# rlorenzo/facet

Hardware: AMD Instinct MI355X
Metric: images/sec whole-node (TOPIQ+SAMP+CLIP+InsightFace ensemble), 1024² batch (higher is better)
Workload: dtype f32

## Files before the change

### facet_amd/csrc/capi.hip

```cpp
#include "capi_internal.h"

static std::string g_create_err;

extern "C" {

const char* fe_version(void) { return "facet_amd 0.1 (gfx950)"; }

int fe_create(int device, size_t arena_bytes, fe_ctx** out) {
  if (!out) return FE_ERR_INVALID;
  *out = nullptr;
  try {
    int ndev = 0;
    hipError_t e = hipGetDeviceCount(&ndev);
    if (e != hipSuccess || ndev <= 0) throw Error(std::string("no HIP device available: ") + hipGetErrorString(e));
    FE_CHECK(device >= 0 && device < ndev, "device %d out of range (%d devices)", device, ndev);
    FE_HIP(hipSetDevice(device));
    hipDeviceProp_t prop;
    FE_HIP(hipGetDeviceProperties(&prop, device));
    FE_CHECK(std::string(prop.gcnArchName).rfind("gfx950", 0) == 0, "device %d is %s; this engine is built for gfx950 only",
             device, prop.gcnArchName);
    auto* x = new fe_ctx();
    x->c.device = device;
    FE_HIP(hipStreamCreateWithFlags(&x->c.stream, hipStreamNonBlocking));
    if (!arena_bytes) {
      size_t free_b = 0, total_b = 0;
      FE_HIP(hipMemGetInfo(&free_b, &total_b));
      arena_bytes = std::min<size_t>((size_t)64 << 30, std::max<size_t>((size_t)2 << 30, free_b / 4));
    }
    x->c.arena.init(arena_bytes);
    FE_HIP(hipEventCreate(&x->t0));
    FE_HIP(hipEventCreate(&x->t1));
    *out = x;
  } catch (const std::exception& e) {
    g_create_err = e.what();
    return FE_ERR_RUNTIME;
  }
  return FE_OK;
}

void fe_destroy(fe_ctx* ctx) {
  if (!ctx) return;
  (void)hipSetDevice(ctx->c.device);
  (void)hipStreamSynchronize(ctx->c.stream);
  if (ctx->t0) (void)hipEventDestroy(ctx->t0);
  if (ctx->t1) (void)hipEventDestroy(ctx->t1);
  if (ctx->d_out) (void)hipFree(ctx->d_out);
  if (ctx->d_rec) (void)hipFree(ctx->d_rec);
  for (int i = 0; i < 2; ++i) {
    if (ctx->stage_buf[i]) (void)hipFree(ctx->stage_buf[i]);
    if (ctx->ev_copied[i]) (void)hipEventDestroy(ctx->ev_copied[i]);
    if (ctx->ev_consumed[i]) (void)hipEventDestroy(ctx->ev_consumed[i]);
  }
  if (ctx->copy_stream) (void)hipStreamDestroy(ctx->copy_stream);
  for (void* q : ctx->misc_allocs) (void)hipFree(q);
  if (ctx->clip_in) (void)hipFree(ctx->clip_in);
  if (ctx->samp_in) (void)hipFree(ctx->samp_in);
  delete ctx;
}

const char* fe_last_error(fe_ctx* ctx) { return ctx ? ctx->c.err.c_str() : g_create_err.c_str(); }

int fe_sync(fe_ctx* ctx) {
  return fe_api(ctx, [&] {
    FE_HIP(hipStreamSynchronize(ctx->c.stream));
  });
}

int fe_set_microbatch(fe_ctx* ctx, int n) {
  return fe_api(ctx, [&] {
    FE_CHECK(n >= 1 && n <= 256, "microbatch %d out of range", n);
    ctx->microbatch = n;
  });
}

int fe_set_conv_variant(fe_ctx* ctx, int variant) {
  return fe_api(ctx, [&] {
    ctx->c.force_variant = variant;
  });
}

int fe_dev_alloc(fe_ctx* ctx, size_t bytes, void** d_out) {
  return fe_api(ctx, [&] {
    FE_CHECK(d_out != nullptr, "null out");
    FE_HIP(hipSetDevice(ctx->c.device));
    FE_HIP(hipMalloc(d_out, bytes ? bytes : 16));
  });
// ... 245 lines not shown
```

### facet_amd/csrc/capi_internal.h

```cpp
#pragma once
#include "../../include/facet_engine.h"
#include "engine.h"
#include "onnx_graph.h"
#include <algorithm>
#include <cmath>
#include <cstring>
#include <stdexcept>
#include <tuple>
#include <type_traits>

using namespace fe;

struct fe_ctx {
  Ctx c;
  int microbatch = 8;
  hipEvent_t t0 = nullptr, t1 = nullptr;
  hipStream_t copy_stream = nullptr;
  uint8_t* stage_buf[2] = {nullptr, nullptr};
  size_t stage_cap[2] = {0, 0};
  hipEvent_t ev_copied[2] = {nullptr, nullptr}, ev_consumed[2] = {nullptr, nullptr};
  short* warp_wtab = nullptr;
  struct CvResizeTab { int* ofs; short* coef; };
  std::map<std::tuple<int, int, int>, CvResizeTab> cvresize;
  int* hsv_sdiv = nullptr; int* hsv_hdiv = nullptr;
  double* phash_cos = nullptr;
  std::vector<void*> misc_allocs;
  float* clip_in = nullptr;
  size_t clip_in_cap = 0;
  float* samp_in = nullptr;
  size_t samp_in_cap = 0;
  float* d_rec = nullptr;
  size_t d_rec_cap = 0;
  int ensemble_mask = 7;
  float* d_out = nullptr;
  size_t d_out_cap = 0;
  float* out_buf(size_t floats) {
    if (floats > d_out_cap) {
      if (d_out) (void)hipFree(d_out);
      d_out = nullptr; d_out_cap = 0;
      FE_HIP(hipMalloc((void**)&d_out, floats * sizeof(float)));
      d_out_cap = floats;
    }
    return d_out;
  }
};

class ImageStager {
 public:
  ImageStager(fe_ctx* ctx, const uint8_t* imgs, int n, size_t per_image, int mb, int on_device)
      : x_(ctx), imgs_(imgs), n_(n), per_(per_image), mb_(mb), dev_(on_device) {
    if (!dev_) {
      if (!x_->copy_stream) {
        FE_HIP(hipStreamCreateWithFlags(&x_->copy_stream, hipStreamNonBlocking));
        for (int i = 0; i < 2; ++i) {
          FE_HIP(hipEventCreateWithFlags(&x_->ev_copied[i], hipEventDisableTiming));
          FE_HIP(hipEventCreateWithFlags(&x_->ev_consumed[i], hipEventDisableTiming));
        }
      }
      const size_t need = (size_t)std::min(mb_, n_) * per_;
      for (int i = 0; i < 2; ++i)
        if (x_->stage_cap[i] < need) {
          FE_HIP(hipStreamSynchronize(x_->c.stream));
          if (x_->stage_buf[i]) FE_HIP(hipFree(x_->stage_buf[i]));
          x_->stage_buf[i] = nullptr; x_->stage_cap[i] = 0;
          FE_HIP(hipMalloc((void**)&x_->stage_buf[i], need));
          x_->stage_cap[i] = need;
        }
      issue(0);
    }
  }
  int chunks() const { return (n_ + mb_ - 1) / mb_; }
  int count(int k) const { return std::min(mb_, n_ - k * mb_); }
  const uint8_t* get(int k) {
    if (dev_) return imgs_ + (size_t)k * mb_ * per_;
    FE_HIP(hipStreamWaitEvent(x_->c.stream, x_->ev_copied[k & 1], 0));
    return x_->stage_buf[k & 1];
  }
  void done(int k) {
    if (dev_) return;
    FE_HIP(hipEventRecord(x_->ev_consumed[k & 1], x_->c.stream));
    consumed_[k & 1] = true;
    if (k + 1 < chunks()) issue(k + 1);
  }
 private:
  void issue(int k) {
    const int b = k & 1;
    if (consumed_[b]) FE_HIP(hipStreamWaitEvent(x_->copy_stream, x_->ev_consumed[b], 0));
    FE_HIP(hipMemcpyAsync(x_->stage_buf[b], imgs_ + (size_t)k * mb_ * per_, (size_t)count(k) * per_, hipMemcpyHostToDevice,
                          x_->copy_stream));
    FE_HIP(hipEventRecord(x_->ev_copied[b], x_->copy_stream));
  }
  fe_ctx* x_; const uint8_t* imgs_; int n_; size_t per_; int mb_, dev_;
  bool consumed_[2] = {false, false};
};

inline void fe_drain(fe_ctx* ctx) {
  if (ctx->copy_stream) (void)hipStreamSynchronize(ctx->copy_stream);
  if (ctx->c.stream) (void)hipStreamSynchronize(ctx->c.stream);
}

struct CapacityError : std::runtime_error { using std::runtime_error::runtime_error; };

enum class OnError {
  Runtime,
  Capacity,
  VlmCapacity
};
inline bool vlm_capacity_error(const char* msg) {
  return strstr(msg, "arena exhausted") || strstr(msg, "out of memory") || strstr(msg, "do not fit") || strstr(msg, "max_seq <= 8192");
}

template <class F>
int fe_api(fe_ctx* ctx, OnError policy, F&& body) {
  if (!ctx) return FE_ERR_INVALID;
  try {
    (void)hipSetDevice(ctx->c.device);
    if constexpr (std::is_void_v<decltype(body())>) {
      body();
      return FE_OK;
    } else {
      return body();
    }
  } catch (const std::exception& e) {
    ctx->c.err = e.what();
    fe_drain(ctx);
    const bool capacity = (policy == OnError::Capacity && dynamic_cast<const CapacityError*>(&e)) ||
                          (policy == OnError::VlmCapacity && vlm_capacity_error(e.what()));
    return capacity ? FE_ERR_CAPACITY : FE_ERR_RUNTIME;
  }
}
template <class F>
int fe_api(fe_ctx* ctx, F&& body) { return fe_api(ctx, OnError::Runtime, body); }
// ... 31 lines not shown
```

### facet_amd/csrc/capi_models.hip

```cpp
#include "capi_internal.h"

namespace {
const float kImagenetMean[3] = {0.485f, 0.456f, 0.406f};
const float kImagenetStd[3] = {0.229f, 0.224f, 0.225f};
const float kClipMean[3] = {0.48145466f, 0.4578275f, 0.40821073f};
const float kClipStd[3] = {0.26862954f, 0.26130258f, 0.27577711f};

int py_round_half_even(double v) {
  const double f = std::floor(v);
  const double d = v - f;
  if (d > 0.5) return (int)f + 1;
  if (d < 0.5) return (int)f;
  return ((long long)f % 2 == 0) ? (int)f : (int)f + 1;
}

template <class T>
void topiq_backbone_chunk(fe_ctx* ctx, const uint8_t* d_rgb, int nb, int h, int w, std::vector<TensorT<T>>& feats) {
  Ctx& C = ctx->c;
  const int long_edge = h > w ? h : w;
  if (long_edge > 1024) {
    const double sc = 1024.0 / long_edge;
    const int nw = (int)(w * sc), nh = (int)(h * sc);
    uint8_t* small = (uint8_t*)C.arena.alloc((size_t)nb * nh * nw * 3);
    resize_u8(C, d_rgb, nb, h, w, nh, nw, FE_FILTER_LANCZOS, 0, nh, 0, nw, small);
    d_rgb = small; h = nh; w = nw;
  }
  Tensor x = C.arena.tensor(nb, h, w, 4);
  launch_u8_to_nhwc4_norm(d_rgb, x.p, (size_t)nb * h * w, kImagenetMean, kImagenetStd, 0, C.stream);
  resnet_forward<T>(C, ctx->c.topiq->backbone, x, &feats, ctx->c.topiq->dw.res32);
}
void topiq_chunk_score(fe_ctx* ctx, const uint8_t* d_in, int nb, int h, int w, float* d_scores) {
  Ctx& C = ctx->c;
  const bool small = (size_t)h * (size_t)w < C.topiq_f32_below && !C.topiq->dw.half_only && !C.topiq->dw.res32;
// ... 36 lines not shown
  auto samp_on = [&](auto sal) {
    typedef decltype(sal.p) SP;
    typedef std::remove_pointer_t<SP> TS;
    if (!with_samp) return;
    if (C.samp->dw.prec == PREC_BF16) sampnet_forward<bf16, TS>(C, *C.samp, x, sal, pw, at, sd);
    else if (C.samp->dw.prec == PREC_F16) sampnet_forward<f16, TS>(C, *C.samp, x, sal, pw, at, sd);
    else sampnet_forward<float, TS>(C, *C.samp, x, sal, pw, at, sd);
  };
  const int prec = C.u2netp->dw.prec;
  if (prec == PREC_BF16) {
    TensorH sal = C.arena.tensor_t<bf16>(x.n, x.h, x.w, 1);
    u2netp_forward<bf16>(C, *C.u2netp, x, sal);
    samp_on(sal);
    if (d_sal) launch_convert(sal.p, d_sal, sal.numel(), C.stream);
  } else if (prec == PREC_F16) {
    TensorF16 sal = C.arena.tensor_t<f16>(x.n, x.h, x.w, 1);
    u2netp_forward<f16>(C, *C.u2netp, x, sal);
    samp_on(sal);
    if (d_sal) launch_convert(sal.p, d_sal, sal.numel(), C.stream);
  } else {
    Tensor sal = C.arena.tensor(x.n, x.h, x.w, 1);
    u2netp_forward<float>(C, *C.u2netp, x, sal);
    samp_on(sal);
    if (d_sal) FE_HIP(hipMemcpyAsync(d_sal, sal.p, sal.numel() * sizeof(float), hipMemcpyDeviceToDevice, C.stream));
  }
}

void compact_crops(float* buf, size_t per, int c, int left, hipStream_t s) {
  for (int done = 0; done < left; done += c) {
    const int n = std::min(c, left - done);
    FE_HIP(hipMemcpyAsync(buf + (size_t)done * per, buf + (size_t)(c + done) * per, (size_t)n * per * sizeof(float), hipMemcpyDeviceToDevice, s));
  }
}
int clip_tower_chunk(const ClipModel& m, int n) {
  if (n <= 40) return n;
  const int hi = std::min(n, 128), lo = std::max(32, hi - 40), ntile = std::max(1, m.width / 128);
  int best = hi;
  double best_eff = 0.0;
  for (int c = hi; c >= lo; --c) {
    const long wgs = (((long)c * m.tokens + 127) / 128) * ntile;
    const double eff = (double)wgs / (double)(((wgs + 255) / 256) * 256);
    if (eff > best_eff + 1e-9) { best_eff = eff; best = c; }
  }
  return best;
}
void clip_tower(Ctx& C, const Tensor& x, float* feat) {
  const bool r32 = C.clip->dw.res32;
  if (C.clip->split3) { clip_forward_split3(C, *C.clip, x, feat); return; }
  if (C.clip->dw.prec == PREC_BF16) { if (r32) clip_forward<bf16, float>(C, *C.clip, x, feat); else clip_forward<bf16>(C, *C.clip, x, feat); }
  else if (C.clip->dw.prec == PREC_F16) { if (r32) clip_forward<f16, float>(C, *C.clip, x, feat); else clip_forward<f16>(C, *C.clip, x, feat); }
  else clip_forward<float>(C, *C.clip, x, feat);
}
class ClipBatcher {
 public:
  ClipBatcher(fe_ctx* ctx, int n_total, int max_push, float* d_feat, float* d_norm, float* d_aes)
      : x_(ctx), feat_(d_feat), norm_(d_norm), aes_(d_aes) {
    const ClipModel& m = *ctx->c.clip;
    hw_ = m.patch_size * (int)std::lround(std::sqrt((double)(m.tokens - 1)));
    od_ = m.out_dim;
    per_ = (size_t)hw_ * hw_ * 4;
    chunk_ = clip_tower_chunk(m, n_total);
    const size_t need = (size_t)(chunk_ + max_push) * per_;
    if (ctx->clip_in_cap < need) {
      FE_HIP(hipStreamSynchronize(ctx->c.stream));
      if (ctx->clip_in) FE_HIP(hipFree(ctx->clip_in));
      ctx->clip_in = nullptr; ctx->clip_in_cap = 0;
      FE_HIP(hipMalloc((void**)&ctx->clip_in, need * sizeof(float)));
      ctx->clip_in_cap = need;
    }
  }
  void push(const Tensor& xt) {
    FE_CHECK(xt.c == 4 && xt.ld == 4 && xt.h == hw_ && xt.w == hw_, "clip batcher: crop layout");
    FE_HIP(hipMemcpyAsync(x_->clip_in + (size_t)count_ * per_, xt.p, (size_t)xt.n * per_ * sizeof(float), hipMemcpyDeviceToDevice, x_->c.stream));
    count_ += xt.n;
    while (count_ >= chunk_) run(chunk_);
  }
  void finish() {
    while (count_ > 0) run(std::min(count_, chunk_));
  }
 private:
  void run(int c) {
    Ctx& C = x_->c;
    const size_t mark = C.arena.mark();
    Tensor x;
    x.p = x_->clip_in; x.n = c; x.h = hw_; x.w = hw_; x.c = 4; x.ld = 4;
    clip_tower(C, x, feat_ + (size_t)done_ * od_);
    if (norm_) l2_normalize(C, feat_ + (size_t)done_ * od_, norm_ + (size_t)done_ * od_, c, od_);
    if (aes_) aesthetic_forward(C, *C.aesthetic, feat_ + (size_t)done_ * od_, c, aes_ + done_);
    C.arena.rewind(mark);
    const int left = count_ - c;
    compact_crops(x_->clip_in, per_, c, left, C.stream);
    done_ += c;
    count_ = left;
  }
  fe_ctx* x_;
  float *feat_, *norm_, *aes_;
  int hw_ = 224, od_ = 768, chunk_ = 1, count_ = 0, done_ = 0;
  size_t per_ = 0;
};
class SampBatcher {
 public:
  SampBatcher(fe_ctx* ctx, int n_total, int max_push, float* pw, float* at, float* sd) : x_(ctx), pw_(pw), at_(at), sd_(sd) {
    const size_t room = ctx->c.arena.capacity() > ((size_t)8 << 30) ? ctx->c.arena.capacity() - ((size_t)8 << 30) : ctx->c.arena.capacity() / 4;
    const int fit = (int)std::min<size_t>(128, std::max<size_t>(1, room / ((size_t)150 << 20)));
    chunk_ = std::max(1, std::min(n_total, std::max(fit, std::min(max_push, 32))));
    per_ = (size_t)224 * 224 * 4;
    const size_t need = (size_t)(chunk_ + max_push) * per_;
    if (ctx->samp_in_cap < need) {
      FE_HIP(hipStreamSynchronize(ctx->c.stream));
      if (ctx->samp_in) FE_HIP(hipFree(ctx->samp_in));
      ctx->samp_in = nullptr; ctx->samp_in_cap = 0;
      FE_HIP(hipMalloc((void**)&ctx->samp_in, need * sizeof(float)));
      ctx->samp_in_cap = need;
    }
  }
  void push(const Tensor& xt) {
    FE_CHECK(xt.c == 4 && xt.ld == 4 && xt.h == 224 && xt.w == 224, "samp batcher: crop layout");
    FE_HIP(hipMemcpyAsync(x_->samp_in + (size_t)count_ * per_, xt.p, (size_t)xt.n * per_ * sizeof(float), hipMemcpyDeviceToDevice, x_->c.stream));
    count_ += xt.n;
    while (count_ >= chunk_) run(chunk_);
  }
  void finish() {
    while (count_ > 0) run(std::min(count_, chunk_));
  }
 private:
  void run(int c) {
    Ctx& C = x_->c;
    const size_t mark = C.arena.mark();
    Tensor x;
    x.p = x_->samp_in; x.n = c; x.h = 224; x.w = 224; x.c = 4; x.ld = 4;
    samp_chunk(x_, x, true, pw_ + (size_t)done_ * 8, at_ + (size_t)done_ * 6, sd_ + (size_t)done_ * 5, nullptr);
    C.arena.rewind(mark);
    const int left = count_ - c;
    compact_crops(x_->samp_in, per_, c, left, C.stream);
    done_ += c;
    count_ = left;
  }
  fe_ctx* x_;
  float *pw_, *at_, *sd_;
  int chunk_ = 1, count_ = 0, done_ = 0;
  size_t per_ = 0;
};

__global__ void records_interleave_kernel(const float* __restrict__ planes, size_t n4, int n, float* __restrict__ rec, int ld) {
  const size_t i = (size_t)blockIdx.x * blockDim.x + threadIdx.x;
  if (i >= (size_t)n * FE_RECORD_FLOATS) return;
  const int img = (int)(i / FE_RECORD_FLOATS), f = (int)(i - (size_t)img * FE_RECORD_FLOATS);
  const size_t o_aes = n4, o_pw = 2 * n4, o_at = o_pw + 8 * n4, o_sd = o_at + 6 * n4, o_emb = o_sd + 5 * n4;
  float v;
  if (f == 0) v = planes[img];
  else if (f == 1) v = planes[o_aes + img];
  else if (f < 10) v = planes[o_pw + (size_t)img * 8 + (f - 2)];
  else if (f < 16) v = planes[o_at + (size_t)img * 6 + (f - 10)];
  else if (f < 21) v = planes[o_sd + (size_t)img * 5 + (f - 16)];
  else v = planes[o_emb + (size_t)img * 768 + (f - 21)];
  rec[(size_t)img * ld + f] = v;
}

int ensemble_run(fe_ctx* ctx, const uint8_t* rgb, int n, int h, int w, int on_device, float* d_rec, int ld) {
  Ctx& C = ctx->c;
  const size_t per = (size_t)h * w * 3;
  const size_t n4 = ((size_t)n + 3) & ~(size_t)3;
  const size_t o_aes = n4, o_pw = 2 * n4, o_at = o_pw + 8 * n4, o_sd = o_at + 6 * n4, o_emb = o_sd + 5 * n4,
               o_feat = o_emb + 768 * n4, total = o_feat + 768 * n4;
  float* d_pl = ctx->out_buf(total);
  FE_HIP(hipMemsetAsync(d_pl, 0, total * sizeof(float), C.stream));
  const int sel = ctx->ensemble_mask;
  const bool do_topiq = (sel & 1) && C.topiq && C.topiq->has_head, do_clip = (sel & 2) && C.clip, do_samp = (sel & 4) && C.samp && C.u2netp;
  float* p_topiq = d_pl;  float* p_aes = d_pl + o_aes;  float* p_pw = d_pl + o_pw;  float* p_at = d_pl + o_at;
  float* p_sd = d_pl + o_sd;  float* p_emb = d_pl + o_emb;  float* d_feat = d_pl + o_feat;
  std::unique_ptr<ClipBatcher> tower;
  if (do_clip) tower = std::make_unique<ClipBatcher>(ctx, n, ctx->microbatch, d_feat, p_emb, C.aesthetic ? p_aes : nullptr);
  std::unique_ptr<SampBatcher> samp;
  if (do_samp) samp = std::make_unique<SampBatcher>(ctx, n, ctx->microbatch, p_pw, p_at, p_sd);
  ImageStager st(ctx, rgb, n, per, ctx->microbatch, on_device);
  for (int k = 0; k < st.chunks(); ++k) {
    const int i0 = k * ctx->microbatch, nb = st.count(k);
    C.arena.reset();
    const uint8_t* d_in = st.get(k);
    if (do_topiq) {
      const size_t mark = C.arena.mark();
      topiq_chunk_score(ctx, d_in, nb, h, w, p_topiq + i0);
      C.arena.rewind(mark);
    }
    if (do_clip) {
      const size_t mark = C.arena.mark();
      Tensor xt = preprocess_square224(C, d_in, nb, h, w, FE_FILTER_BICUBIC, true, kClipMean, kClipStd, 0);
      tower->push(xt);
      C.arena.rewind(mark);
    }
    if (do_samp) {
      const size_t mark = C.arena.mark();
      Tensor xt = preprocess_square224(C, d_in, nb, h, w, FE_FILTER_BILINEAR, false, kImagenetMean, kImagenetStd, 0);
      samp->push(xt);
      C.arena.rewind(mark);
    }
    st.done(k);
  }
  if (tower) tower->finish();
  if (samp) samp->finish();
  const size_t work = (size_t)n * FE_RECORD_FLOATS;
  hipLaunchKernelGGL(records_interleave_kernel, dim3((unsigned)((work + 255) / 256)), dim3(256), 0, C.stream, d_pl, n4, n, d_rec, ld);
  FE_HIP(hipGetLastError());
  return (do_topiq ? 1 : 0) | (do_clip ? 2 : 0) | (do_samp ? 4 : 0);
}
}

extern "C" {

int fe_topiq_feature_shape(int h, int w, int level, int dims[3]) {
  if (!dims || h < 32 || w < 32 || level < 0 || level > 4) return FE_ERR_INVALID;
  const int long_edge = h > w ? h : w;
  if (long_edge > 1024) {
    const double sc = 1024.0 / long_edge;
    w = (int)(w * sc); h = (int)(h * sc);
  }
  static const int ch[5] = {64, 256, 512, 1024, 2048};
  int fh = conv_out_dim(h, 7, 2, 3, 1), fw = conv_out_dim(w, 7, 2, 3, 1);
  if (level >= 1) { fh = conv_out_dim(fh, 3, 2, 1, 1); fw = conv_out_dim(fw, 3, 2, 1, 1); }
  for (int l = 2; l <= level; ++l) { fh = conv_out_dim(fh, 3, 2, 1, 1); fw = conv_out_dim(fw, 3, 2, 1, 1); }
  dims[0] = ch[level]; dims[1] = fh; dims[2] = fw;
  return FE_OK;
}

int fe_topiq_features(fe_ctx* ctx, const uint8_t* rgb, int n, int h, int w, int on_device, int level, float* out) {
  return fe_api(ctx, [&] {
    Ctx& C = ctx->c;
    if (!C.topiq) { C.err = "topiq weights not loaded"; return FE_ERR_NOT_LOADED; }
    FE_CHECK(rgb && out && n > 0 && h >= 32 && w >= 32 && level >= 0 && level <= 4, "bad arguments");
    const size_t img_bytes = (size_t)h * w * 3;
    size_t out_per_img = 0;
    for (int i0 = 0; i0 < n; i0 += ctx->microbatch) {
      const int nb = std::min(ctx->microbatch, n - i0);
      C.arena.reset();
      const uint8_t* d_in = resident(C, rgb + (size_t)i0 * img_bytes, nb * img_bytes, on_device);
      if (C.topiq->dw.prec == PREC_BF16) {
// ... 89 lines not shown
}

int fe_aesthetic_score(fe_ctx* ctx, const float* feats, int n, float* aesthetic_raw) {
  return fe_api(ctx, [&] {
    Ctx& C = ctx->c;
    if (!C.aesthetic) { C.err = "aesthetic head weights not loaded"; return FE_ERR_NOT_LOADED; }
    FE_CHECK(feats && aesthetic_raw && n > 0, "bad arguments");
    const int d = 768;
    for (int i0 = 0; i0 < n; i0 += 65536) {
      const int nb = std::min(65536, n - i0);
      C.arena.reset();
      float* d_in = upload(C, feats + (size_t)i0 * d, (size_t)nb * d);
      float* d_out = (float*)C.arena.alloc((size_t)nb * sizeof(float));
      aesthetic_forward(C, *C.aesthetic, d_in, nb, d_out);
      FE_HIP(hipMemcpyAsync(aesthetic_raw + i0, d_out, (size_t)nb * sizeof(float), hipMemcpyDeviceToHost, C.stream));
      FE_HIP(hipStreamSynchronize(C.stream));
    }
    return FE_OK;
  });
}

int fe_clip_encode_image(fe_ctx* ctx, const float* x, int n, int on_device, float* features, float* emb_norm,
                         float* aesthetic_raw) {
  return fe_api(ctx, [&] {
    Ctx& C = ctx->c;
    if (!C.clip) { C.err = "clip weights not loaded"; return FE_ERR_NOT_LOADED; }
    if (aesthetic_raw && !C.aesthetic) { C.err = "aesthetic head weights not loaded"; return FE_ERR_NOT_LOADED; }
    FE_CHECK(x && n > 0 && (features || emb_norm || aesthetic_raw), "bad arguments");
    const int hw = C.clip->patch_size * (int)std::lround(std::sqrt((double)(C.clip->tokens - 1)));
    const int od = C.clip->out_dim;
    const size_t per = (size_t)3 * hw * hw;
    float* d_out = ctx->out_buf((size_t)n * (2 * od + 1));
    float* d_feat = d_out; float* d_norm = d_out + (size_t)n * od; float* d_aes = d_out + (size_t)n * 2 * od;
    const int step = clip_tower_chunk(*C.clip, n);
    for (int i0 = 0; i0 < n; i0 += step) {
      const int nb = std::min(step, n - i0);
      C.arena.reset();
      Tensor xt;
      if (on_device) {
        xt = C.arena.tensor(nb, hw, hw, 4);
        launch_nchw_to_nhwc(x + (size_t)i0 * per, xt.p, nb, 3, hw, hw, 4, C.stream);
      } else {
        xt = upload_nchw(C, x + (size_t)i0 * per, nb, 3, hw, hw, 4);
      }
      clip_tower(C, xt, d_feat + (size_t)i0 * od);
      if (emb_norm) l2_normalize(C, d_feat + (size_t)i0 * od, d_norm + (size_t)i0 * od, nb, od);
      if (aesthetic_raw) aesthetic_forward(C, *C.aesthetic, d_feat + (size_t)i0 * od, nb, d_aes + i0);
    }
    if (features) FE_HIP(hipMemcpyAsync(features, d_feat, (size_t)n * od * sizeof(float), hipMemcpyDeviceToHost, C.stream));
    if (emb_norm) FE_HIP(hipMemcpyAsync(emb_norm, d_norm, (size_t)n * od * sizeof(float), hipMemcpyDeviceToHost, C.stream));
    if (aesthetic_raw) FE_HIP(hipMemcpyAsync(aesthetic_raw, d_aes, (size_t)n * sizeof(float), hipMemcpyDeviceToHost, C.stream));
    FE_HIP(hipStreamSynchronize(C.stream));
    return FE_OK;
  });
}

int fe_clip_encode_images(fe_ctx* ctx, const uint8_t* rgb, int n, int h, int w, int on_device, float* features,
                          float* emb_norm, float* aesthetic_raw) {
  return fe_api(ctx, [&] {
    Ctx& C = ctx->c;
    if (!C.clip) { C.err = "clip weights not loaded"; return FE_ERR_NOT_LOADED; }
    if (aesthetic_raw && !C.aesthetic) { C.err = "aesthetic head weights not loaded"; return FE_ERR_NOT_LOADED; }
    FE_CHECK(rgb && n > 0 && h > 0 && w > 0, "bad arguments");
    const int od = C.clip->out_dim;
    const size_t per = (size_t)h * w * 3;
    float* d_out = ctx->out_buf((size_t)n * (2 * od + 1));
    float* d_feat = d_out; float* d_norm = d_out + (size_t)n * od; float* d_aes = d_out + (size_t)n * 2 * od;
// ... 130 lines not shown
```

### facet_amd/csrc/fe_common.h

```cpp
#pragma once
#include <hip/hip_runtime.h>
#include "fe_check.h"
#include <cstdint>
#include <cstdio>
#include <atomic>
#include <cstring>
#include <map>
#include <mutex>
#include <stdexcept>
#include <string>
#include <vector>

namespace fe {


#define FE_HIP(expr)                                                                      \
  do {                                                                                    \
    hipError_t _e = (expr);                                                               \
    if (_e != hipSuccess) {                                                               \
      char _b[512];                                                                       \
      snprintf(_b, sizeof _b, "%s:%d: %s -> %s", __FILE__, __LINE__, #expr,               \
               hipGetErrorString(_e));                                                    \
      throw fe::Error(_b);                                                                \
    }                                                                                     \
  } while (0)

inline void ensure_dynamic_lds(const void* kernel, size_t bytes, std::atomic<uint64_t>& done) {
  int dev = 0;
  FE_HIP(hipGetDevice(&dev));
  const uint64_t bit = 1ull << (dev & 63);
  if (done.load(std::memory_order_acquire) & bit) return;
  FE_HIP(hipFuncSetAttribute(kernel, hipFuncAttributeMaxDynamicSharedMemorySize, (int)bytes));
  done.fetch_or(bit, std::memory_order_release);
}

enum Act : int { ACT_NONE = 0, ACT_RELU = 1, ACT_GELU = 2, ACT_SIGMOID = 3, ACT_PRELU = 4, ACT_SOFTPLUS = 5, ACT_QUICKGELU = 6 };

__device__ __forceinline__ float fe_apply_act(float v, int act) {
  if (act == ACT_RELU) return v > 0.f ? v : 0.f;
  if (act == ACT_GELU) return 0.5f * v * (1.f + erff(v * 0.70710678118654752440f));
  if (act == ACT_SIGMOID) return 1.f / (1.f + __expf(-v));
  if (act == ACT_SOFTPLUS) return v > 20.f ? v : log1pf(expf(v));
  if (act == ACT_QUICKGELU) return v / (1.f + __expf(-1.702f * v));
// ... 104 lines not shown
  float4 v;
  fe_unpack2(p, u.x, v.x, v.y); fe_unpack2(p, u.y, v.z, v.w);
  return v;
}
__device__ __forceinline__ void st4(float* p, float4 v) { *reinterpret_cast<float4*>(p) = v; }
__device__ __forceinline__ void st4(f16* p, float4 v) {
  *reinterpret_cast<uint2*>(p) = make_uint2(fe_pack2(p, v.x, v.y), fe_pack2(p, v.z, v.w));
}
__device__ __forceinline__ void st4(bf16* p, float4 v) {
  typedef __bf16 bf4 __attribute__((ext_vector_type(4)));
  bf4 o; o[0] = (bf16)v.x; o[1] = (bf16)v.y; o[2] = (bf16)v.z; o[3] = (bf16)v.w;
  *reinterpret_cast<bf4*>(p) = o;
}

class Arena {
 public:
  void init(size_t bytes) {
    release();
    FE_HIP(hipMalloc(&base_, bytes));
    cap_ = bytes;
    off_ = 0;
  }
  void release() {
    if (base_) (void)hipFree(base_);
    base_ = nullptr;
    cap_ = off_ = 0;
  }
  ~Arena() { release(); }
  void reset() { off_ = 0; }
  size_t mark() const { return off_; }
  void rewind(size_t m) { off_ = m; }
  size_t capacity() const { return cap_; }
  size_t high_water() const { return high_; }
  void* alloc(size_t bytes) {
    size_t a = (off_ + 255) & ~(size_t)255;
    FE_CHECK(a + bytes <= cap_, "arena exhausted: need %zu at %zu of %zu", bytes, a, cap_);
    off_ = a + bytes;
    if (off_ > high_) high_ = off_;
    return (char*)base_ + a;
  }
  template <class T>
  TensorT<T> tensor_t(int n, int h, int w, int c) {
    TensorT<T> t;
    t.n = n; t.h = h; t.w = w; t.c = c; t.ld = c;
    t.p = (T*)alloc(t.numel() * sizeof(T));
    return t;
  }
  Tensor tensor(int n, int h, int w, int c) { return tensor_t<float>(n, h, w, c); }
  template <class T>
  T* array(size_t count) { return (T*)alloc(count * sizeof(T)); }
 private:
  void* base_ = nullptr;
  size_t cap_ = 0, off_ = 0, high_ = 0;
};

template <class T>
struct ConvParamsT {
  const T* x; int ldx;
  const T* w;
  const float* scale;
  const float* shift;
  const float* slope;
  const T* res; int ldr;
  const T* gate; int ldg;
  T* y; int ldy;
  int N, H, W, Cin, Ho, Wo, Cout;
// ... 203 lines not shown
```

Before: 236.2.

## Overlap CLIP/SAMP towers with TOPIQ on a second stream via op plan

Introduces a planned op schedule that puts CLIP (when not f32) and SAMP crop preprocessing and tower runs on a side stream with its own arena, while TOPIQ runs on the main stream, joined by events. Copy-in staging buffers are released only after both lanes have read them. The goal is to fill the GPU with concurrent independent model work instead of serializing the ensemble. It costs a second arena allocation and extra event synchronization, and the two lanes now compete for compute and memory.

```diff
diff --git a/facet_amd/csrc/capi.hip b/facet_amd/csrc/capi.hip
--- a/facet_amd/csrc/capi.hip
+++ b/facet_amd/csrc/capi.hip
@@ -52,6 +52,13 @@
     if (ctx->ev_consumed[i]) (void)hipEventDestroy(ctx->ev_consumed[i]);
   }
   if (ctx->copy_stream) (void)hipStreamDestroy(ctx->copy_stream);
+  if (ctx->side.stream) {
+    (void)hipStreamSynchronize(ctx->side.stream);
+    (void)hipStreamDestroy(ctx->side.stream);
+  }
+  for (hipEvent_t e : {ctx->side.ev_start, ctx->side.ev_join, ctx->side.ev_read[0], ctx->side.ev_read[1]})
+    if (e) (void)hipEventDestroy(e);
+  ctx->side.arena.release();
   for (void* q : ctx->misc_allocs) (void)hipFree(q);
   if (ctx->clip_in) (void)hipFree(ctx->clip_in);
   if (ctx->samp_in) (void)hipFree(ctx->samp_in);
diff --git a/facet_amd/csrc/capi_internal.h b/facet_amd/csrc/capi_internal.h
--- a/facet_amd/csrc/capi_internal.h
+++ b/facet_amd/csrc/capi_internal.h
@@ -32,6 +32,11 @@
   float* d_rec = nullptr;
   size_t d_rec_cap = 0;
   int ensemble_mask = 7;
+  struct SideLane {
+    hipStream_t stream = nullptr;
+    Arena arena;
+    hipEvent_t ev_start = nullptr, ev_join = nullptr, ev_read[2] = {nullptr, nullptr};
+  } side;
   float* d_out = nullptr;
   size_t d_out_cap = 0;
   float* out_buf(size_t floats) {
@@ -50,24 +55,26 @@
   ImageStager(fe_ctx* ctx, const uint8_t* imgs, int n, size_t per_image, int mb, int on_device)
       : x_(ctx), imgs_(imgs), n_(n), per_(per_image), mb_(mb), dev_(on_device) {
     if (!dev_) {
-      if (!x_->copy_stream) {
-        FE_HIP(hipStreamCreateWithFlags(&x_->copy_stream, hipStreamNonBlocking));
-        for (int i = 0; i < 2; ++i) {
-          FE_HIP(hipEventCreateWithFlags(&x_->ev_copied[i], hipEventDisableTiming));
-          FE_HIP(hipEventCreateWithFlags(&x_->ev_consumed[i], hipEventDisableTiming));
-        }
-      }
-      const size_t need = (size_t)std::min(mb_, n_) * per_;
-      for (int i = 0; i < 2; ++i)
-        if (x_->stage_cap[i] < need) {
-          FE_HIP(hipStreamSynchronize(x_->c.stream));
-          if (x_->stage_buf[i]) FE_HIP(hipFree(x_->stage_buf[i]));
-          x_->stage_buf[i] = nullptr; x_->stage_cap[i] = 0;
-          FE_HIP(hipMalloc((void**)&x_->stage_buf[i], need));
-          x_->stage_cap[i] = need;
-        }
+      prepare(x_, (size_t)std::min(mb_, n_) * per_);
       issue(0);
     }
+  }
+  static void prepare(fe_ctx* x, size_t need) {
+    if (!x->copy_stream) {
+      FE_HIP(hipStreamCreateWithFlags(&x->copy_stream, hipStreamNonBlocking));
+      for (int i = 0; i < 2; ++i) {
+        FE_HIP(hipEventCreateWithFlags(&x->ev_copied[i], hipEventDisableTiming));
+        FE_HIP(hipEventCreateWithFlags(&x->ev_consumed[i], hipEventDisableTiming));
+      }
+    }
+    for (int i = 0; i < 2; ++i)
+      if (x->stage_cap[i] < need) {
+        FE_HIP(hipStreamSynchronize(x->c.stream));
+        if (x->stage_buf[i]) FE_HIP(hipFree(x->stage_buf[i]));
+        x->stage_buf[i] = nullptr; x->stage_cap[i] = 0;
+        FE_HIP(hipMalloc((void**)&x->stage_buf[i], need));
+        x->stage_cap[i] = need;
+      }
   }
   int chunks() const { return (n_ + mb_ - 1) / mb_; }
   int count(int k) const { return std::min(mb_, n_ - k * mb_); }
@@ -96,8 +103,24 @@
 
 inline void fe_drain(fe_ctx* ctx) {
   if (ctx->copy_stream) (void)hipStreamSynchronize(ctx->copy_stream);
+  if (ctx->side.stream) (void)hipStreamSynchronize(ctx->side.stream);
   if (ctx->c.stream) (void)hipStreamSynchronize(ctx->c.stream);
 }
+
+class LaneScope {
+ public:
+  explicit LaneScope(fe_ctx* ctx, bool on_side) : x_(on_side ? ctx : nullptr) { flip(); }
+  ~LaneScope() { flip(); }
+  LaneScope(const LaneScope&) = delete;
+  LaneScope& operator=(const LaneScope&) = delete;
+ private:
+  void flip() {
+    if (!x_) return;
+    std::swap(x_->c.stream, x_->side.stream);
+    x_->c.arena.swap(x_->side.arena);
+  }
+  fe_ctx* x_;
+};
 
 struct CapacityError : std::runtime_error { using std::runtime_error::runtime_error; };
 
diff --git a/facet_amd/csrc/capi_models.hip b/facet_amd/csrc/capi_models.hip
--- a/facet_amd/csrc/capi_models.hip
+++ b/facet_amd/csrc/capi_models.hip
@@ -1,4 +1,5 @@
 #include "capi_internal.h"
+#include "ensemble_plan.h"
 
 namespace {
 const float kImagenetMean[3] = {0.485f, 0.456f, 0.406f};
@@ -101,18 +102,6 @@
     FE_HIP(hipMemcpyAsync(buf + (size_t)done * per, buf + (size_t)(c + done) * per, (size_t)n * per * sizeof(float), hipMemcpyDeviceToDevice, s));
   }
 }
-int clip_tower_chunk(const ClipModel& m, int n) {
-  if (n <= 40) return n;
-  const int hi = std::min(n, 128), lo = std::max(32, hi - 40), ntile = std::max(1, m.width / 128);
-  int best = hi;
-  double best_eff = 0.0;
-  for (int c = hi; c >= lo; --c) {
-    const long wgs = (((long)c * m.tokens + 127) / 128) * ntile;
-    const double eff = (double)wgs / (double)(((wgs + 255) / 256) * 256);
-    if (eff > best_eff + 1e-9) { best_eff = eff; best = c; }
-  }
-  return best;
-}
 void clip_tower(Ctx& C, const Tensor& x, float* feat) {
   const bool r32 = C.clip->dw.res32;
   if (C.clip->split3) { clip_forward_split3(C, *C.clip, x, feat); return; }
@@ -128,7 +117,7 @@
     hw_ = m.patch_size * (int)std::lround(std::sqrt((double)(m.tokens - 1)));
     od_ = m.out_dim;
     per_ = (size_t)hw_ * hw_ * 4;
-    chunk_ = clip_tower_chunk(m, n_total);
+    chunk_ = clip_tower_chunk(m.width, m.tokens, n_total);
     const size_t need = (size_t)(chunk_ + max_push) * per_;
     if (ctx->clip_in_cap < need) {
       FE_HIP(hipStreamSynchronize(ctx->c.stream));
@@ -138,40 +127,49 @@
       ctx->clip_in_cap = need;
     }
   }
-  void push(const Tensor& xt) {
+  int chunk() const { return chunk_; }
+  void stage(const Tensor& xt, int slot) {
     FE_CHECK(xt.c == 4 && xt.ld == 4 && xt.h == hw_ && xt.w == hw_, "clip batcher: crop layout");
-    FE_HIP(hipMemcpyAsync(x_->clip_in + (size_t)count_ * per_, xt.p, (size_t)xt.n * per_ * sizeof(float), hipMemcpyDeviceToDevice, x_->c.stream));
-    count_ += xt.n;
-    while (count_ >= chunk_) run(chunk_);
-  }
-  void finish() {
-    while (count_ > 0) run(std::min(count_, chunk_));
-  }
- private:
-  void run(int c) {
+    FE_CHECK((size_t)(slot + xt.n) * per_ <= x_->clip_in_cap, "clip batcher: slot %d + %d past the staging buffer", slot, xt.n);
+    FE_HIP(hipMemcpyAsync(x_->clip_in + (size_t)slot * per_, xt.p, (size_t)xt.n * per_ * sizeof(float), hipMemcpyDeviceToDevice, x_->c.stream));
+  }
+  void run(int c, int done) {
     Ctx& C = x_->c;
     const size_t mark = C.arena.mark();
     Tensor x;
     x.p = x_->clip_in; x.n = c; x.h = hw_; x.w = hw_; x.c = 4; x.ld = 4;
-    clip_tower(C, x, feat_ + (size_t)done_ * od_);
-    if (norm_) l2_normalize(C, feat_ + (size_t)done_ * od_, norm_ + (size_t)done_ * od_, c, od_);
-    if (aes_) aesthetic_forward(C, *C.aesthetic, feat_ + (size_t)done_ * od_, c, aes_ + done_);
+    clip_tower(C, x, feat_ + (size_t)done * od_);
+    if (norm_) l2_normalize(C, feat_ + (size_t)done * od_, norm_ + (size_t)done * od_, c, od_);
+    if (aes_) aesthetic_forward(C, *C.aesthetic, feat_ + (size_t)done * od_, c, aes_ + done);
     C.arena.rewind(mark);
-    const int left = count_ - c;
-    compact_crops(x_->clip_in, per_, c, left, C.stream);
+  }
+  void compact(int c, int left) { compact_crops(x_->clip_in, per_, c, left, x_->c.stream); }
+  void push(const Tensor& xt) {
+    stage(xt, count_);
+    count_ += xt.n;
+    while (count_ >= chunk_) consume(chunk_);
+  }
+  void finish() {
+    while (count_ > 0) consume(std::min(count_, chunk_));
+  }
+ private:
+  void consume(int c) {
+    run(c, done_);
+    compact(c, count_ - c);
     done_ += c;
-    count_ = left;
+    count_ -= c;
   }
   fe_ctx* x_;
   float *feat_, *norm_, *aes_;
   int hw_ = 224, od_ = 768, chunk_ = 1, count_ = 0, done_ = 0;
   size_t per_ = 0;
 };
+constexpr size_t kSampBytesPerImage = (size_t)150 << 20;
 class SampBatcher {
  public:
   SampBatcher(fe_ctx* ctx, int n_total, int max_push, float* pw, float* at, float* sd) : x_(ctx), pw_(pw), at_(at), sd_(sd) {
     const size_t room = ctx->c.arena.capacity() > ((size_t)8 << 30) ? ctx->c.arena.capacity() - ((size_t)8 << 30) : ctx->c.arena.capacity() / 4;
-    const int fit = (int)std::min<size_t>(128, std::max<size_t>(1, room / ((size_t)150 << 20)));
+    const int fit = (int)std::min<size_t>(128, std::max<size_t>(1, room / kSampBytesPerImage));
     chunk_ = std::max(1, std::min(n_total, std::max(fit, std::min(max_push, 32))));
     per_ = (size_t)224 * 224 * 4;
     const size_t need = (size_t)(chunk_ + max_push) * per_;
@@ -183,27 +181,35 @@
       ctx->samp_in_cap = need;
     }
   }
-  void push(const Tensor& xt) {
+  int chunk() const { return chunk_; }
+  void stage(const Tensor& xt, int slot) {
     FE_CHECK(xt.c == 4 && xt.ld == 4 && xt.h == 224 && xt.w == 224, "samp batcher: crop layout");
-    FE_HIP(hipMemcpyAsync(x_->samp_in + (size_t)count_ * per_, xt.p, (size_t)xt.n * per_ * sizeof(float), hipMemcpyDeviceToDevice, x_->c.stream));
-    count_ += xt.n;
-    while (count_ >= chunk_) run(chunk_);
-  }
-  void finish() {
-    while (count_ > 0) run(std::min(count_, chunk_));
-  }
- private:
-  void run(int c) {
+    FE_CHECK((size_t)(slot + xt.n) * per_ <= x_->samp_in_cap, "samp batcher: slot %d + %d past the staging buffer", slot, xt.n);
+    FE_HIP(hipMemcpyAsync(x_->samp_in + (size_t)slot * per_, xt.p, (size_t)xt.n * per_ * sizeof(float), hipMemcpyDeviceToDevice, x_->c.stream));
+  }
+  void run(int c, int done) {
     Ctx& C = x_->c;
     const size_t mark = C.arena.mark();
     Tensor x;
     x.p = x_->samp_in; x.n = c; x.h = 224; x.w = 224; x.c = 4; x.ld = 4;
-    samp_chunk(x_, x, true, pw_ + (size_t)done_ * 8, at_ + (size_t)done_ * 6, sd_ + (size_t)done_ * 5, nullptr);
+    samp_chunk(x_, x, true, pw_ + (size_t)done * 8, at_ + (size_t)done * 6, sd_ + (size_t)done * 5, nullptr);
     C.arena.rewind(mark);
-    const int left = count_ - c;
-    compact_crops(x_->samp_in, per_, c, left, C.stream);
+  }
+  void compact(int c, int left) { compact_crops(x_->samp_in, per_, c, left, x_->c.stream); }
+  void push(const Tensor& xt) {
+    stage(xt, count_);
+    count_ += xt.n;
+    while (count_ >= chunk_) consume(chunk_);
+  }
+  void finish() {
+    while (count_ > 0) consume(std::min(count_, chunk_));
+  }
+ private:
+  void consume(int c) {
+    run(c, done_);
+    compact(c, count_ - c);
     done_ += c;
-    count_ = left;
+    count_ -= c;
   }
   fe_ctx* x_;
   float *pw_, *at_, *sd_;
@@ -226,14 +232,37 @@
   rec[(size_t)img * ld + f] = v;
 }
 
+bool side_lane_ready(fe_ctx* ctx, size_t need) {
+  auto& s = ctx->side;
+  try {
+    if (!s.stream) FE_HIP(hipStreamCreateWithFlags(&s.stream, hipStreamNonBlocking));
+    for (hipEvent_t* e : {&s.ev_start, &s.ev_join, &s.ev_read[0], &s.ev_read[1]})
+      if (!*e) FE_HIP(hipEventCreateWithFlags(e, hipEventDisableTiming));
+    if (s.arena.capacity() < need) {
+      FE_HIP(hipStreamSynchronize(s.stream));
+      s.arena.init(need);
+    }
+    return true;
+  } catch (const std::exception&) {
+    (void)hipGetLastError();
+    return false;
+  }
+}
+size_t side_arena_bytes(fe_ctx* ctx, int mb, int h, int w, int clip_chunk, int samp_chunk) {
+  const size_t tower = std::max((size_t)clip_chunk * ((size_t)32 << 20), (size_t)samp_chunk * kSampBytesPerImage);
+  const size_t ow = w <= h ? 224 : (size_t)(224.0 * w / h) + 1;
+  const size_t pre = (size_t)mb * ((size_t)h * ow * 3 + (size_t)224 * 224 * (3 + 16) + 1024);
+  return std::min(ctx->c.arena.capacity(), tower + pre + ((size_t)64 << 20));
+}
+
 int ensemble_run(fe_ctx* ctx, const uint8_t* rgb, int n, int h, int w, int on_device, float* d_rec, int ld) {
+  using namespace fe::plan;
   Ctx& C = ctx->c;
   const size_t per = (size_t)h * w * 3;
   const size_t n4 = ((size_t)n + 3) & ~(size_t)3;
   const size_t o_aes = n4, o_pw = 2 * n4, o_at = o_pw + 8 * n4, o_sd = o_at + 6 * n4, o_emb = o_sd + 5 * n4,
                o_feat = o_emb + 768 * n4, total = o_feat + 768 * n4;
   float* d_pl = ctx->out_buf(total);
-  FE_HIP(hipMemsetAsync(d_pl, 0, total * sizeof(float), C.stream));
   const int sel = ctx->ensemble_mask;
   const bool do_topiq = (sel & 1) && C.topiq && C.topiq->has_head, do_clip = (sel & 2) && C.clip, do_samp = (sel & 4) && C.samp && C.u2netp;
   float* p_topiq = d_pl;  float* p_aes = d_pl + o_aes;  float* p_pw = d_pl + o_pw;  float* p_at = d_pl + o_at;
@@ -242,35 +271,79 @@
   if (do_clip) tower = std::make_unique<ClipBatcher>(ctx, n, ctx->microbatch, d_feat, p_emb, C.aesthetic ? p_aes : nullptr);
   std::unique_ptr<SampBatcher> samp;
   if (do_samp) samp = std::make_unique<SampBatcher>(ctx, n, ctx->microbatch, p_pw, p_at, p_sd);
-  ImageStager st(ctx, rgb, n, per, ctx->microbatch, on_device);
-  for (int k = 0; k < st.chunks(); ++k) {
-    const int i0 = k * ctx->microbatch, nb = st.count(k);
-    C.arena.reset();
-    const uint8_t* d_in = st.get(k);
-    if (do_topiq) {
-      const size_t mark = C.arena.mark();
-      topiq_chunk_score(ctx, d_in, nb, h, w, p_topiq + i0);
-      C.arena.rewind(mark);
-    }
-    if (do_clip) {
-      const size_t mark = C.arena.mark();
-      Tensor xt = preprocess_square224(C, d_in, nb, h, w, FE_FILTER_BICUBIC, true, kClipMean, kClipStd, 0);
-      tower->push(xt);
-      C.arena.rewind(mark);
-    }
-    if (do_samp) {
-      const size_t mark = C.arena.mark();
-      Tensor xt = preprocess_square224(C, d_in, nb, h, w, FE_FILTER_BILINEAR, false, kImagenetMean, kImagenetStd, 0);
-      samp->push(xt);
-      C.arena.rewind(mark);
-    }
-    st.done(k);
-  }
-  if (tower) tower->finish();
-  if (samp) samp->finish();
-  const size_t work = (size_t)n * FE_RECORD_FLOATS;
-  hipLaunchKernelGGL(records_interleave_kernel, dim3((unsigned)((work + 255) / 256)), dim3(256), 0, C.stream, d_pl, n4, n, d_rec, ld);
-  FE_HIP(hipGetLastError());
+  if (!on_device) ImageStager::prepare(ctx, (size_t)std::min(ctx->microbatch, n) * per);
+
+  Shape sh;
+  sh.n = n; sh.mb = ctx->microbatch; sh.on_device = on_device != 0;
+  sh.topiq = do_topiq; sh.clip = do_clip; sh.samp = do_samp;
+  sh.clip_chunk = tower ? tower->chunk() : 1;
+  sh.samp_chunk = samp ? samp->chunk() : 1;
+  sh.clip_side = do_clip && C.clip->dw.prec != PREC_F32;
+  if (const char* v = getenv("FE_OVERLAP_LANES")) {
+    sh.samp_side = strcmp(v, "clip") != 0;
+    sh.clip_side = strcmp(v, "samp") != 0;
+    sh.samp_first = strcmp(v, "samp_first") == 0;
+  }
+  const bool side_clip = do_clip && sh.clip_side, side_samp = do_samp && sh.samp_side;
+  sh.overlap = (side_clip || side_samp) && !C.profile && getenv("FE_NO_OVERLAP") == nullptr &&
+               side_lane_ready(ctx, side_arena_bytes(ctx, std::min(ctx->microbatch, n), h, w, side_clip ? sh.clip_chunk : 0, side_samp ? sh.samp_chunk : 0));
+
+  const hipStream_t lane[N_LANES] = {C.stream, ctx->side.stream, ctx->copy_stream};
+  hipEvent_t event[N_EVENTS];
+  event[EV_START] = ctx->side.ev_start; event[EV_JOIN] = ctx->side.ev_join;
+  for (int b = 0; b < 2; ++b) {
+    event[EV_COPIED0 + b] = ctx->ev_copied[b]; event[EV_CONSUMED0 + b] = ctx->ev_consumed[b]; event[EV_SIDE_READ0 + b] = ctx->side.ev_read[b];
+  }
+  auto input = [&](int k) { return on_device ? rgb + (size_t)k * ctx->microbatch * per : (const uint8_t*)ctx->stage_buf[k & 1]; };
+  for (const Op& o : build(sh)) {
+    LaneScope scope(ctx, o.lane == LANE_SIDE);
+    switch (o.kind) {
+      case OP_CLEAR:
+        FE_HIP(hipMemsetAsync(d_pl, 0, total * sizeof(float), lane[LANE_MAIN]));
+        break;
+      case OP_COPY_IN:
+        FE_HIP(hipMemcpyAsync(ctx->stage_buf[o.mb & 1], rgb + (size_t)o.img0 * per, (size_t)o.count * per, hipMemcpyHostToDevice, lane[LANE_COPY]));
+        break;
+      case OP_RECORD:
+        FE_HIP(hipEventRecord(event[o.event], lane[o.lane]));
+        break;
+      case OP_WAIT:
+        FE_HIP(hipStreamWaitEvent(lane[o.lane], event[o.event], 0));
+        break;
+      case OP_TOPIQ:
+        C.arena.reset();
+        topiq_chunk_score(ctx, input(o.mb), o.count, h, w, p_topiq + o.img0);
+        break;
+      case OP_CLIP_PRE:
+        C.arena.reset();
+        tower->stage(preprocess_square224(C, input(o.mb), o.count, h, w, FE_FILTER_BICUBIC, true, kClipMean, kClipStd, 0), o.slot);
+        break;
+      case OP_CLIP_TOWER:
+        C.arena.reset();
+        tower->run(o.count, o.img0);
+        break;
+      case OP_CLIP_COMPACT:
+        tower->compact(o.count, o.left);
+        break;
+      case OP_SAMP_PRE:
+        C.arena.reset();
+        samp->stage(preprocess_square224(C, input(o.mb), o.count, h, w, FE_FILTER_BILINEAR, false, kImagenetMean, kImagenetStd, 0), o.slot);
+        break;
+      case OP_SAMP_NETS:
+        C.arena.reset();
+        samp->run(o.count, o.img0);
+        break;
+      case OP_SAMP_COMPACT:
+        samp->compact(o.count, o.left);
+        break;
+      case OP_INTERLEAVE: {
+        const size_t work = (size_t)n * FE_RECORD_FLOATS;
+        hipLaunchKernelGGL(records_interleave_kernel, dim3((unsigned)((work + 255) / 256)), dim3(256), 0, lane[LANE_MAIN], d_pl, n4, n, d_rec, ld);
+        FE_HIP(hipGetLastError());
+        break;
+      }
+    }
+  }
   return (do_topiq ? 1 : 0) | (do_clip ? 2 : 0) | (do_samp ? 4 : 0);
 }
 }
@@ -426,7 +499,7 @@
     const size_t per = (size_t)3 * hw * hw;
     float* d_out = ctx->out_buf((size_t)n * (2 * od + 1));
     float* d_feat = d_out; float* d_norm = d_out + (size_t)n * od; float* d_aes = d_out + (size_t)n * 2 * od;
-    const int step = clip_tower_chunk(*C.clip, n);
+    const int step = clip_tower_chunk(C.clip->width, C.clip->tokens, n);
     for (int i0 = 0; i0 < n; i0 += step) {
       const int nb = std::min(step, n - i0);
       C.arena.reset();
diff --git a/facet_amd/csrc/ensemble_plan.h b/facet_amd/csrc/ensemble_plan.h
--- /dev/null
+++ b/facet_amd/csrc/ensemble_plan.h
@@ -0,0 +1,163 @@
+#pragma once
+#include <algorithm>
+#include <vector>
+
+namespace fe {
+
+inline int clip_tower_chunk(int width, int tokens, int n) {
+  if (n <= 40) return n;
+  const int hi = std::min(n, 128), lo = std::max(32, hi - 40), ntile = std::max(1, width / 128);
+  int best = hi;
+  double best_eff = 0.0;
+  for (int c = hi; c >= lo; --c) {
+    const long wgs = (((long)c * tokens + 127) / 128) * ntile;
+    const double eff = (double)wgs / (double)(((wgs + 255) / 256) * 256);
+    if (eff > best_eff + 1e-9) { best_eff = eff; best = c; }
+  }
+  return best;
+}
+
+namespace plan {
+
+enum Lane : int { LANE_MAIN = 0, LANE_SIDE = 1, LANE_COPY = 2, N_LANES = 3 };
+enum Kind : int {
+  OP_CLEAR,
+  OP_COPY_IN,
+  OP_TOPIQ,
+  OP_CLIP_PRE,
+  OP_CLIP_TOWER,
+  OP_CLIP_COMPACT,
+  OP_SAMP_PRE, OP_SAMP_NETS, OP_SAMP_COMPACT,
+  OP_RECORD, OP_WAIT,
+  OP_INTERLEAVE
+};
+enum Region : int { R_STAGE0, R_STAGE1, R_CLIP_IN, R_SAMP_IN, R_OUT_TOPIQ, R_OUT_CLIP, R_OUT_SAMP, R_ARENA_MAIN, R_ARENA_SIDE };
+enum Event : int { EV_START, EV_JOIN, EV_COPIED0, EV_COPIED1, EV_CONSUMED0, EV_CONSUMED1, EV_SIDE_READ0, EV_SIDE_READ1, N_EVENTS };
+
+struct Access { int region, lo, hi; bool write; };
+struct Op {
+  int kind = OP_CLEAR, lane = LANE_MAIN;
+  int mb = 0, img0 = 0, count = 0;
+  int slot = 0, left = 0;
+  int event = -1;
+  Access acc[3];
+  int n_acc = 0;
+  void touch(int region, int lo, int hi, bool write) { acc[n_acc++] = Access{region, lo, hi, write}; }
+};
+
+struct Shape {
+  int n = 0, mb = 1;
+  int clip_chunk = 1, samp_chunk = 1;
+  bool on_device = true;
+  bool topiq = true, clip = true, samp = true;
+  bool overlap = true;
+  bool clip_side = true, samp_side = true, samp_first = false;
+};
+
+class Builder {
+ public:
+  explicit Builder(const Shape& s) : s_(s), side_(s.overlap && ((s.clip && s.clip_side) || (s.samp && s.samp_side)) ? LANE_SIDE : LANE_MAIN) {}
+  std::vector<Op> build() {
+    const bool two = side_ == LANE_SIDE;
+    const int chunks = (s_.n + s_.mb - 1) / s_.mb;
+    Op clr = op(OP_CLEAR, LANE_MAIN);
+    clr.touch(R_OUT_TOPIQ, 0, s_.n, true); clr.touch(R_OUT_CLIP, 0, s_.n, true); clr.touch(R_OUT_SAMP, 0, s_.n, true);
+    ops_.push_back(clr);
+    if (two) { sync(OP_RECORD, LANE_MAIN, EV_START); sync(OP_WAIT, LANE_SIDE, EV_START); }
+    if (!s_.on_device) copy_in(0);
+    for (int k = 0; k < chunks; ++k) {
+      const int b = k & 1;
+      if (!s_.on_device) {
+        sync(OP_WAIT, LANE_MAIN, EV_COPIED0 + b);
+        if (two) sync(OP_WAIT, LANE_SIDE, EV_COPIED0 + b);
+      }
+      if (!two) topiq(k);
+      if (s_.samp && s_.samp_first) crops(k, OP_SAMP_PRE, R_SAMP_IN, R_OUT_SAMP, s_.samp_chunk, samp_);
+      if (s_.clip) crops(k, OP_CLIP_PRE, R_CLIP_IN, R_OUT_CLIP, s_.clip_chunk, clip_);
+      if (s_.samp && !s_.samp_first) crops(k, OP_SAMP_PRE, R_SAMP_IN, R_OUT_SAMP, s_.samp_chunk, samp_);
+      if (two && !s_.on_device) sync(OP_RECORD, LANE_SIDE, EV_SIDE_READ0 + b);
+      if (two) topiq(k);
+      if (!s_.on_device) {
+        sync(OP_RECORD, LANE_MAIN, EV_CONSUMED0 + b);
+        if (k + 1 < chunks) copy_in(k + 1);
+      }
+    }
+    if (s_.samp && s_.samp_first) while (samp_.count > 0) run(OP_SAMP_PRE, R_SAMP_IN, R_OUT_SAMP, std::min(samp_.count, s_.samp_chunk), samp_);
+    if (s_.clip) while (clip_.count > 0) run(OP_CLIP_PRE, R_CLIP_IN, R_OUT_CLIP, std::min(clip_.count, s_.clip_chunk), clip_);
+    if (s_.samp && !s_.samp_first) while (samp_.count > 0) run(OP_SAMP_PRE, R_SAMP_IN, R_OUT_SAMP, std::min(samp_.count, s_.samp_chunk), samp_);
+    if (two) { sync(OP_RECORD, LANE_SIDE, EV_JOIN); sync(OP_WAIT, LANE_MAIN, EV_JOIN); }
+    Op il = op(OP_INTERLEAVE, LANE_MAIN);
+    il.count = s_.n;
+    il.touch(R_OUT_TOPIQ, 0, s_.n, false); il.touch(R_OUT_CLIP, 0, s_.n, false); il.touch(R_OUT_SAMP, 0, s_.n, false);
+    ops_.push_back(il);
+    return ops_;
+  }
+
+ private:
+  struct Gather { int count = 0, done = 0; };
+  Op op(int kind, int lane) const { Op o; o.kind = kind; o.lane = lane; return o; }
+  int nb(int k) const { return std::min(s_.mb, s_.n - k * s_.mb); }
+  int arena(int lane) const { return lane == LANE_SIDE ? R_ARENA_SIDE : R_ARENA_MAIN; }
+  int lane_of(int pre) const { return (pre == OP_CLIP_PRE ? s_.clip_side : s_.samp_side) ? side_ : (int)LANE_MAIN; }
+  void sync(int kind, int lane, int event) { Op o = op(kind, lane); o.event = event; ops_.push_back(o); }
+  void copy_in(int k) {
+    const int b = k & 1;
+    if (k >= 2) {
+      sync(OP_WAIT, LANE_COPY, EV_CONSUMED0 + b);
+      if (side_ == LANE_SIDE) sync(OP_WAIT, LANE_COPY, EV_SIDE_READ0 + b);
+    }
+    Op o = op(OP_COPY_IN, LANE_COPY);
+    o.mb = k; o.img0 = k * s_.mb; o.count = nb(k);
+    o.touch(R_STAGE0 + b, 0, nb(k), true);
+    ops_.push_back(o);
+    sync(OP_RECORD, LANE_COPY, EV_COPIED0 + b);
+  }
+  void topiq(int k) {
+    if (!s_.topiq) return;
+    Op o = op(OP_TOPIQ, LANE_MAIN);
+    o.mb = k; o.img0 = k * s_.mb; o.count = nb(k);
+    if (!s_.on_device) o.touch(R_STAGE0 + (k & 1), 0, nb(k), false);
+    o.touch(R_OUT_TOPIQ, o.img0, o.img0 + o.count, true);
+    o.touch(R_ARENA_MAIN, 0, 1, true);
+    ops_.push_back(o);
+  }
+  void crops(int k, int pre, int staging, int out, int chunk, Gather& g) {
+    const int lane = lane_of(pre);
+    Op o = op(pre, lane);
+    o.mb = k; o.img0 = k * s_.mb; o.count = nb(k); o.slot = g.count;
+    if (!s_.on_device) o.touch(R_STAGE0 + (k & 1), 0, nb(k), false);
+    o.touch(staging, g.count, g.count + o.count, true);
+    o.touch(arena(lane), 0, 1, true);
+    ops_.push_back(o);
+    g.count += o.count;
+    while (g.count >= chunk) run(pre, staging, out, chunk, g);
+  }
+  void run(int pre, int staging, int out, int c, Gather& g) {
+    const int lane = lane_of(pre);
+    Op o = op(pre + 1, lane);
+    o.img0 = g.done; o.count = c;
+    o.touch(staging, 0, c, false);
+    o.touch(out, g.done, g.done + c, true);
+    o.touch(arena(lane), 0, 1, true);
+    ops_.push_back(o);
+    const int left = g.count - c;
+    if (left > 0) {
+      Op m = op(pre + 2, lane);
+      m.count = c; m.left = left;
+      m.touch(staging, c, c + left, false);
+      m.touch(staging, 0, left, true);
+      ops_.push_back(m);
+    }
+    g.done += c;
+    g.count = left;
+  }
+  Shape s_;
+  int side_;
+  Gather clip_, samp_;
+  std::vector<Op> ops_;
+};
+
+inline std::vector<Op> build(const Shape& s) { return Builder(s).build(); }
+
+}
+}
diff --git a/facet_amd/csrc/fe_common.h b/facet_amd/csrc/fe_common.h
--- a/facet_amd/csrc/fe_common.h
+++ b/facet_amd/csrc/fe_common.h
@@ -9,6 +9,7 @@
 #include <mutex>
 #include <stdexcept>
 #include <string>
+#include <utility>
 #include <vector>
 
 namespace fe {
@@ -179,6 +180,7 @@
   void rewind(size_t m) { off_ = m; }
   size_t capacity() const { return cap_; }
   size_t high_water() const { return high_; }
+  void swap(Arena& o) { std::swap(base_, o.base_); std::swap(cap_, o.cap_); std::swap(off_, o.off_); std::swap(high_, o.high_); }
   void* alloc(size_t bytes) {
     size_t a = (off_ + 255) & ~(size_t)255;
     FE_CHECK(a + bytes <= cap_, "arena exhausted: need %zu at %zu of %zu", bytes, a, cap_);
```

After: 239.3, median of 6. +1.3%, better.
